# davelailai/DS-GCN

Hardware: AMD Instinct MI355X
Metric: clips/sec fwd+bwd, DS-STGCN NTU-60 3x64x25x2 (higher is better)
Workload: dtype f32

## Files before the change

ds-gcn_amd/csrc/tmsplit.hip:

```cpp
#include <algorithm>

#include "common.h"
#include "bn_jobs.h"

namespace {

constexpr int TS_NT = 256;
constexpr int TS_MAXBR = 8;
constexpr int TS_OOB = 0x7ffffff0;
constexpr int TS_R = 4, TS_H = 4;

typedef float f32x2s __attribute__((ext_vector_type(2)));
typedef unsigned u32x4s __attribute__((ext_vector_type(4)));

struct TSBranch {
  int type;
  int c0, bc, dil;
  const float* w;
  const float* b;
  float* dwp;
  float* dbp;
};

struct TSArgs {
  const float* z; const float* zaug; const float* scale; const float* shift;
  const float* coeff;
  float* f; float* oaug; float* stats;
  const float* ge; const float* doaug;
  float* dz; float* dzaug; float* part;
  int n_act, n, C, T, Tout, V, nbr, ngrp, ngrpa, nconv, eplanes, sboff, haw, splits, pstride;
  int cw[TS_MAXBR];
  int ngroups, gfirst[TS_MAXBR], gcount[TS_MAXBR];
  int exp;
  TSBranch br[TS_MAXBR];
};

__device__ __forceinline__ __amdgpu_buffer_rsrc_t ts_rsrc(const void* p, size_t bytes) {
  return __builtin_amdgcn_make_buffer_rsrc(const_cast<void*>(p), (short)0, (int)bytes, 0x00020000);
}
__device__ __forceinline__ f32x4 ts_load4(__amdgpu_buffer_rsrc_t r, int voff, int soff) {
  return __builtin_bit_cast(f32x4, __builtin_amdgcn_raw_buffer_load_b128(r, voff, soff, 0));
}
__device__ __forceinline__ f32x2s ts_load2(__amdgpu_buffer_rsrc_t r, int voff, int soff) {
  return __builtin_bit_cast(f32x2s, __builtin_amdgcn_raw_buffer_load_b64(r, voff, soff, 0));
}
__device__ __forceinline__ void ts_store4(f32x4 v, __amdgpu_buffer_rsrc_t r, int voff) {
  __builtin_amdgcn_raw_buffer_store_b128(__builtin_bit_cast(u32x4s, v), r, voff, 0, 0);
}
__device__ __forceinline__ int ts_row32(int r, int half) { return (r & 3) + 8 * (r >> 2) + 4 * half; }
__device__ __forceinline__ int ts_rowoff(bool ok, int base, int rowoff) {
  return (int)((unsigned)(ok ? base : TS_OOB) + (unsigned)rowoff);
}
__device__ __forceinline__ int ts_cp(int bc) { return (min(64, max(bc, 1)) + 7) & ~7; }

__device__ __forceinline__ const TSBranch& ts_conv_window(const TSArgs& a, int w) { return a.br[a.cw[w]]; }

template <typename ACC>
__device__ __forceinline__ ACC ts_rowread(const float* Tw, int half, int l31) {
  const f32x4* rowp = reinterpret_cast<const f32x4*>(Tw + l31 * 36 + half * 16);
  ACC s = 0;
#pragma unroll
  for (int q = 0; q < 4; ++q) {
    const f32x4 v = rowp[q];
    s += ((ACC)v.x + (ACC)v.y) + ((ACC)v.z + (ACC)v.w);
  }
  return s;
}


#ifdef DSGCN_LAB
__device__ long long g_tsc_stamp[16];
__device__ int g_tsc_block = 0;
#define TSC_STAMP() do { if (!AUG && (int)blockIdx.x == g_tsc_block && threadIdx.x == 0 && nst < 14) g_tsc_stamp[nst++] = wall_clock64(); } while (0)
#else
#define TSC_STAMP() do {} while (0)
#endif

template <bool FWD, int MT, bool ODD, bool AUG, bool S2 = false>
__device__ __forceinline__ void ts_conv(const TSArgs& a, const TSBranch& br, bool first, float* lds, int grp, int lane, int wave) {
  constexpr int KT = 3, PDK = 2, NS = KT * PDK;
  constexpr bool FOLD = FWD && !AUG;
  constexpr int FP = 32;
  static_assert(!(S2 && ODD), "stride 2 has its own load forms");
// ... 832 lines not shown
      if (a.br[i].type == 0)
        for (int k = lane; k < a.br[i].bc * 2; k += 64) tab[((size_t)(a.ngrp + n) * a.C + a.br[i].c0) * 2 + k] = 0.f;
  }
  const int per = S2 ? a.T * a.V + a.Tout * a.V + ((a.T + 3) & ~3) + ((a.Tout + 3) & ~3) + 32
                     : (FWD ? 1 : 2) * a.T * a.V + 2 * ((a.T + 3) & ~3) + 32;
  for (int i = 0; i < a.nbr; ++i) {
    if (a.br[i].type == 0) continue;
    if (c < a.br[i].bc) {
      if constexpr (S2) ts_elem2<FWD>(a, a.br[i], lds + (size_t)wave * per, n, c, lane);
      else ts_elem<FWD>(a, a.br[i], lds + (size_t)wave * per, n, c, lane);
      return;
    }
    c -= a.br[i].bc;
  }
}

__global__ __launch_bounds__(64) void k_tsp_prep(const float* __restrict__ gf, const float* __restrict__ f,
                                                 const float* __restrict__ oaug, const float* __restrict__ coeff,
                                                 const float* __restrict__ A0, const float* __restrict__ B0,
                                                 float* __restrict__ ge, float* __restrict__ doaug,
                                                 float* __restrict__ pcoef, int C, int T, int V) {
  extern __shared__ __attribute__((aligned(16))) float lds[];
  const int lane = threadIdx.x;
  const long plane = blockIdx.x;
  const int c = (int)(plane % C);
  const int L = T * V, L4n = L >> 2, Tp = (T + 3) & ~3;
  float* gl = lds;
  float* ol = lds + L;
  float* cf = ol + Tp;
  if (lane < V) cf[lane] = coeff[lane];
  for (int t = lane; t < T; t += 64) ol[t] = oaug[plane * T + t];
  const float a0 = A0 ? A0[c] : 0.f, b0 = B0 ? B0[c] : 0.f;
  const f32x4* g4 = gf ? reinterpret_cast<const f32x4*>(gf + plane * L) : nullptr;
  const f32x4* f4 = reinterpret_cast<const f32x4*>(f + plane * L);
  f32x4* o4 = reinterpret_cast<f32x4*>(ge + plane * L);
  f32x4* l4 = reinterpret_cast<f32x4*>(gl);
  const f32x4 zero4 = {0.f, 0.f, 0.f, 0.f};
  for (int base = 0; base < L4n; base += 256) {
    f32x4 gv[4], fv[4];
#pragma unroll
    for (int q = 0; q < 4; ++q) {
      const int i = base + q * 64 + lane;
      const bool ok = i < L4n;
      gv[q] = (ok && g4) ? g4[i] : zero4;
      fv[q] = (ok && A0) ? f4[i] : zero4;
    }
#pragma unroll
    for (int q = 0; q < 4; ++q) {
      const int i = base + q * 64 + lane;
      if (i < L4n) {
        f32x4 r;
#pragma unroll
        for (int k = 0; k < 4; ++k) r[k] = gv[q][k] + fmaf(b0, fv[q][k], a0);
        o4[i] = r;
        l4[i] = r;
      }
    }
  }
  wave_lds_sync();
  for (int t = lane; t < T; t += 64) {
    float acc = 0.f;
    for (int v = 0; v < V; ++v) acc = fmaf(gl[t * V + v], cf[v], acc);
    doaug[plane * T + t] = acc;
  }
  {
    const int v = lane & 31, hf = lane >> 5;
    float acc = 0.f;
    if (v < V)
      for (int t = hf; t < T; t += 2) acc = fmaf(gl[t * V + v], ol[t], acc);
    acc += __shfl_xor(acc, 32, 64);
    if (lane < V) pcoef[plane * V + lane] = acc;
  }
}

__host__ __device__ inline int tsw_ls(int w) { return ((w + 1) & ~3) + 2; }

#ifdef DSGCN_LAB
__device__ long long g_tsw_stamp[64];
#define TSW_STAMP() do { if (blockIdx.x == 0 && blockIdx.y == 0 && threadIdx.x == 0 && nst < 62) g_tsw_stamp[nst++] = wall_clock64(); } while (0)
#else
#define TSW_STAMP() do {} while (0)
#endif

template <int CH>
__global__ __launch_bounds__(TS_NT, CH == 32 ? 2 : 1) void k_tspw(TSArgs a, BnCoefTable jobs) {
  constexpr int KT = 3;
  constexpr int JD = CH == 32 ? 4 : 7, JX = CH == 32 ? 10 : 20;
  extern __shared__ __attribute__((aligned(16))) float lds[];
  if ((int)blockIdx.x >= a.splits) {
    if (blockIdx.y == 0)
      bnj_dispatch(jobs, (int)blockIdx.x - a.splits,
                   [&](const BnCoefJob& J, int b) { bn_coef_rows_block<TS_NT>(J, b, reinterpret_cast<double (*)[8][2]>(lds)); });
    return;
  }
#ifdef DSGCN_LAB
  int nst = 0;
#endif
  TSW_STAMP();
  const int tid = threadIdx.x, lane = tid & 63;
  const int wave = __builtin_amdgcn_readfirstlane(tid >> 6);
  const int half = lane >> 5, l31 = lane & 31;
  const int gw0 = a.gfirst[blockIdx.y], gcnt = a.gcount[blockIdx.y];
  const TSBranch& br = ts_conv_window(a, gw0);
  const int V = a.V, T = a.T, L = T * V, C = a.C;
  int bc = 0, ldil = br.dil;
  for (int w = 0; w < gcnt; ++w) {
    const TSBranch& bw = ts_conv_window(a, gw0 + w);
    if (l31 >= bc) ldil = bw.dil;
    bc += bw.bc;
  }
  const int GM = TS_R * V, XM = (TS_R + 2 * TS_H) * V;
  const int GS4 = GM >> 2, XS4 = XM >> 2, SEG4 = (TS_H * V) >> 2;
  const int LSd = tsw_ls(GM + TS_R), LSx = tsw_ls(XM + TS_R + 2 * TS_H);
  float* Ds = lds;
  float* Xs = lds + CH * LSd;
  f32x2s* SB = reinterpret_cast<f32x2s*>(Xs + CH * LSx);
  const f32x2s sb0 = (tid < CH && tid < bc) ? f32x2s{a.scale ? a.scale[br.c0 + tid] : 1.f, a.shift ? a.shift[br.c0 + tid] : 0.f}
                                            : f32x2s{0.f, 0.f};
  const int rel0 = br.c0;

  const int units = a.n * (T / TS_R);
  const int per = (units + a.splits - 1) / a.splits;
  const int u0 = blockIdx.x * per, u1 = min(units, u0 + per);

  const __amdgpu_buffer_rsrc_t rg = ts_rsrc(a.ge, (size_t)a.n * C * L * 4);
  const __amdgpu_buffer_rsrc_t rz = ts_rsrc(a.z, (size_t)a.n * C * L * 4);
  const __amdgpu_buffer_rsrc_t rga = ts_rsrc(a.doaug, (size_t)a.n * C * T * 4);
  const __amdgpu_buffer_rsrc_t rza = ts_rsrc(a.zaug, (size_t)a.n * C * T * 4);
  int vD[JD], lD[JD], vX[JX], lX[JX];
#pragma unroll
  for (int j = 0; j < JD; ++j) {
    const int f = tid + TS_NT * j, row = f / GS4, c4 = f - row * GS4;
    const bool ok = row < bc;
    vD[j] = ok ? (row * L + 4 * c4) * 4 : TS_OOB;
    lD[j] = ok ? row * LSd + 4 * c4 : -1;
  }
#pragma unroll
  for (int j = 0; j < JX; ++j) {
    const int f = tid + TS_NT * j, row = f / XS4, c4 = f - row * XS4;
    const bool ok = row < bc;
    vX[j] = ok ? (row * L + 4 * c4) * 4 : TS_OOB;
    const int seg = c4 / SEG4;
    lX[j] = (row * LSx + 4 * c4) | ((seg == 0 ? 1 : seg == 2 ? 2 : 0) << 20) | ((row & 63) << 22) | (ok ? 1 << 28 : 0);
  }
  const int arow = tid / 3, aseg = tid - arow * 3;
  const bool aokD = tid < CH && tid < bc && !(a.exp & 256), aokX = tid < 3 * CH && arow < bc && !(a.exp & 256);
  const int aneed = aseg == 0 ? 1 : aseg == 2 ? 2 : 0;
  f32x4 gr[JD], xr[JX], ga, xa;
  float dsum[JD], dsa = 0.f;
#pragma unroll
  for (int j = 0; j < JD; ++j) dsum[j] = 0.f;
  int inval = 0;
  auto issue = [&](int u) {
    const int n = u / (T / TS_R), t0 = (u - n * (T / TS_R)) * TS_R;
    const int sg = ((n * C + br.c0) * L + t0 * V) * 4;
    const int sx = ((n * C + br.c0) * L + (t0 - TS_H) * V) * 4;
    inval = (t0 >= TS_H ? 0 : 1) | (t0 + TS_R < T ? 0 : 2);
#pragma unroll
    for (int j = 0; j < JD; ++j) gr[j] = ts_load4(rg, vD[j], sg);
#pragma unroll
    for (int j = 0; j < JX; ++j) {
      const bool ok = (((lX[j] >> 20) & 3) & inval) == 0;
      xr[j] = ts_load4(rz, ok ? vX[j] + sx : TS_OOB, 0);
    }
    ga = ts_load4(rga, aokD ? ((n * C + br.c0 + tid) * T + t0) * 4 : TS_OOB, 0);
    const bool oka = aokX & ((aneed & inval) == 0);
    xa = ts_load4(rza, oka ? ((n * C + br.c0 + arow) * T + t0 + (aseg - 1) * TS_H) * 4 : TS_OOB, 0);
  };
  const bool noact = a.exp & 128;
  auto act = [&](float x, f32x2s sb, bool rl) -> float {
    if (noact) return x;
    const float y = fmaf(x, sb.x, sb.y);
    return rl ? fmaxf(y, 0.f) : y;
  };
  auto commit = [&]() {
#pragma unroll
    for (int j = 0; j < JD; ++j) {
      if (lD[j] >= 0) {
        f32x2s* d = reinterpret_cast<f32x2s*>(Ds + lD[j]);
        d[0] = f32x2s{gr[j].x, gr[j].y};
        d[1] = f32x2s{gr[j].z, gr[j].w};
        dsum[j] += (gr[j].x + gr[j].y) + (gr[j].z + gr[j].w);
      }
    }
#pragma unroll
    for (int j = 0; j < JX; ++j) {
      if (lX[j] & (1 << 28)) {
        const bool ok = (((lX[j] >> 20) & 3) & inval) == 0;
        const int row = (lX[j] >> 22) & 63;
        const f32x2s sb = SB[row];
        const bool rl = rel0 + row < a.n_act;
        f32x2s* d = reinterpret_cast<f32x2s*>(Xs + (lX[j] & 0xfffff));
        d[0] = ok ? f32x2s{act(xr[j].x, sb, rl), act(xr[j].y, sb, rl)} : f32x2s{0.f, 0.f};
        d[1] = ok ? f32x2s{act(xr[j].z, sb, rl), act(xr[j].w, sb, rl)} : f32x2s{0.f, 0.f};
      }
    }
    if (aokD) {
      f32x2s* d = reinterpret_cast<f32x2s*>(Ds + tid * LSd + GM);
      d[0] = f32x2s{ga.x, ga.y};
      d[1] = f32x2s{ga.z, ga.w};
      dsa += (ga.x + ga.y) + (ga.z + ga.w);
    }
    if (aokX) {
      const bool ok = (aneed & inval) == 0;
      const f32x2s sb = SB[arow];
      const bool rl = rel0 + arow < a.n_act;
      f32x2s* d = reinterpret_cast<f32x2s*>(Xs + arow * LSx + XM + aseg * TS_H);
      d[0] = ok ? f32x2s{act(xa.x, sb, rl), act(xa.y, sb, rl)} : f32x2s{0.f, 0.f};
      d[1] = ok ? f32x2s{act(xa.z, sb, rl), act(xa.w, sb, rl)} : f32x2s{0.f, 0.f};
    }
  };

  f32x16 acc[KT];
#pragma unroll
  for (int k = 0; k < KT; ++k)
#pragma unroll
    for (int i = 0; i < 16; ++i) acc[k][i] = 0.f;
  const int mt = CH == 64 ? (wave >> 1) : 0, nt = CH == 64 ? (wave & 1) : 0;
  const int g0 = CH == 32 ? (GS4 * wave) / 4 : 0, g1 = CH == 32 ? (GS4 * (wave + 1)) / 4 : GS4;
  const bool augw = CH == 64 || wave == 0;
  const int sh = ldil * V;
  const bool oddsh = gcnt > 1 || ((sh & 1) && !(a.exp & 512));
  const float* Ap = Ds + (32 * mt + l31) * LSd + 2 * half;
  const float* Bp = Xs + (32 * nt + l31) * LSx + TS_H * V + 2 * half;
  const float* Aq = Ds + (32 * mt + l31) * LSd + GM + 2 * half;
  const float* Bq = Xs + (32 * nt + l31) * LSx + XM + TS_H + 2 * half;
  auto mm = [&](f32x2s av, f32x2s b0, f32x2s b1, f32x2s b2) {
    acc[0] = __builtin_amdgcn_mfma_f32_32x32x2f32(av.x, b0.x, acc[0], 0, 0, 0);
    acc[1] = __builtin_amdgcn_mfma_f32_32x32x2f32(av.x, b1.x, acc[1], 0, 0, 0);
    acc[2] = __builtin_amdgcn_mfma_f32_32x32x2f32(av.x, b2.x, acc[2], 0, 0, 0);
    acc[0] = __builtin_amdgcn_mfma_f32_32x32x2f32(av.y, b0.y, acc[0], 0, 0, 0);
    acc[1] = __builtin_amdgcn_mfma_f32_32x32x2f32(av.y, b1.y, acc[1], 0, 0, 0);
    acc[2] = __builtin_amdgcn_mfma_f32_32x32x2f32(av.y, b2.y, acc[2], 0, 0, 0);
  };

  if (u0 < u1) issue(u0);
  {
    f32x4* l4 = reinterpret_cast<f32x4*>(lds);
    for (int i = tid; i < (CH * (LSd + LSx)) >> 2; i += TS_NT) l4[i] = f32x4{0.f, 0.f, 0.f, 0.f};
    if (tid < CH) SB[tid] = sb0;
  }
  __syncthreads();
  TSW_STAMP();
  for (int u = u0; u < u1; ++u) {
    commit();
    asm volatile("s_waitcnt lgkmcnt(0)" ::: "memory");
    __builtin_amdgcn_s_barrier();
    TSW_STAMP();
    if (u + 1 < u1) issue(u + 1);
    TSW_STAMP();
    if (oddsh) {
#pragma unroll 2
      for (int g = g0; g < g1; ++g) {
        const f32x2s av = *reinterpret_cast<const f32x2s*>(Ap + 4 * g);
        const f32x2s b1 = *reinterpret_cast<const f32x2s*>(Bp + 4 * g);
        const f32x2s b0 = {Bp[4 * g - sh], Bp[4 * g - sh + 1]};
        const f32x2s b2 = {Bp[4 * g + sh], Bp[4 * g + sh + 1]};
        mm(av, b0, b1, b2);
      }
    } else {
#pragma unroll 2
      for (int g = g0; g < g1; ++g) {
        const f32x2s av = *reinterpret_cast<const f32x2s*>(Ap + 4 * g);
        const f32x2s b0 = *reinterpret_cast<const f32x2s*>(Bp + 4 * g - sh);
        const f32x2s b1 = *reinterpret_cast<const f32x2s*>(Bp + 4 * g);
        const f32x2s b2 = *reinterpret_cast<const f32x2s*>(Bp + 4 * g + sh);
        mm(av, b0, b1, b2);
      }
    }
    if (augw) {
      const f32x2s av = *reinterpret_cast<const f32x2s*>(Aq);
      const f32x2s b1 = *reinterpret_cast<const f32x2s*>(Bq);
      const f32x2s b0 = {Bq[-ldil], Bq[1 - ldil]};
      const f32x2s b2 = {Bq[ldil], Bq[1 + ldil]};
      mm(av, b0, b1, b2);
    }
    asm volatile("s_waitcnt lgkmcnt(0)" ::: "memory");
    __builtin_amdgcn_s_barrier();
    TSW_STAMP();
  }

  if (CH == 32) {
    float* Rs = lds;
#pragma unroll
    for (int k = 0; k < KT; ++k)
#pragma unroll
      for (int r = 0; r < 16; ++r) Rs[((wave * KT + k) * 32 + ts_row32(r, half)) * 33 + l31] = acc[k][r];
    __syncthreads();
    for (int w = 0, r0 = 0; w < gcnt; ++w) {
      const TSBranch& bw = ts_conv_window(a, gw0 + w);
      const int wb = bw.bc;
      float* dw = bw.dwp + (size_t)blockIdx.x * a.pstride;
      for (int o = tid; o < KT * wb * wb; o += TS_NT) {
        const int co = o / (wb * KT), r2 = o - co * wb * KT, ci = r2 / KT, k = r2 - ci * KT;
        float v = 0.f;
#pragma unroll
        for (int wv = 0; wv < 4; ++wv) v += Rs[((wv * KT + k) * 32 + r0 + co) * 33 + r0 + ci];
        dw[o] = v;
      }
      r0 += wb;
    }
    __syncthreads();
  } else {
    float* dw = br.dwp + (size_t)blockIdx.x * a.pstride;
    const int ci = 32 * nt + l31;
    if (ci < bc) {
#pragma unroll
      for (int r = 0; r < 16; ++r) {
        const int co = 32 * mt + ts_row32(r, half);
        if (co < bc) {
#pragma unroll
          for (int k = 0; k < KT; ++k) dw[((size_t)co * bc + ci) * KT + k] = acc[k][r];
        }
      }
    }
    __syncthreads();
  }
  float* Bs = lds;
#pragma unroll
  for (int j = 0; j < JD; ++j) {
    const int f = tid + TS_NT * j, row = f / GS4, c4 = f - row * GS4;
    if (row < bc) Bs[row * (GS4 + 2) + c4] = dsum[j];
  }
  if (aokD) Bs[tid * (GS4 + 2) + GS4] = dsa;
  __syncthreads();
  if (tid < bc) {
    float v = 0.f;
    for (int c = 0; c <= GS4; ++c) v += Bs[tid * (GS4 + 2) + c];
    int r0 = 0;
    for (int w = 0; w < gcnt; ++w) {
      const TSBranch& bw = ts_conv_window(a, gw0 + w);
      if (tid >= r0 && tid < r0 + bw.bc) bw.dbp[(size_t)blockIdx.x * a.pstride + tid - r0] = v;
      r0 += bw.bc;
    }
  }
#ifdef DSGCN_LAB
  TSW_STAMP();
  if (blockIdx.x == 0 && blockIdx.y == 0 && threadIdx.x == 0) g_tsw_stamp[63] = nst;
#endif
}

template <int CH>
__global__ __launch_bounds__(TS_NT, CH == 32 ? 2 : 1) void k_tspw2(TSArgs a, BnCoefTable jobs) {
  constexpr int KT = 3;
  constexpr int JD = CH == 32 ? 4 : 7, JX = CH == 32 ? 11 : 21, JA = CH == 32 ? 2 : 3;
  extern __shared__ __attribute__((aligned(16))) float lds[];
  if ((int)blockIdx.x >= a.splits) {
    if (blockIdx.y == 0)
      bnj_dispatch(jobs, (int)blockIdx.x - a.splits,
                   [&](const BnCoefJob& J, int b) { bn_coef_rows_block<TS_NT>(J, b, reinterpret_cast<double (*)[8][2]>(lds)); });
    return;
  }
  const int tid = threadIdx.x, lane = tid & 63;
  const int wave = __builtin_amdgcn_readfirstlane(tid >> 6);
  const int half = lane >> 5, l31 = lane & 31;
  const int gw0 = a.gfirst[blockIdx.y], gcnt = a.gcount[blockIdx.y];
  const TSBranch& br = ts_conv_window(a, gw0);
  const int V = a.V, Ti = a.T, To = a.Tout, Li = Ti * V, Lo = To * V, C = a.C;
  int bc = 0;
  for (int w = 0; w < gcnt; ++w) bc += ts_conv_window(a, gw0 + w).bc;
  auto row_dil = [&](int row) -> int {
    int d = br.dil, r0 = 0;
    for (int w = 0; w < gcnt; ++w) {
      const TSBranch& bw = ts_conv_window(a, gw0 + w);
      if (row >= r0) d = bw.dil;
      r0 += bw.bc;
    }
    return d;
  };
  const int GM = TS_R * V;
  const int GS4 = GM >> 2, Q = (V + 3) >> 2;
  const int LSd = tsw_ls(GM + TS_R);
  float* Ds = lds;
  float* Xs = lds + CH * LSd;
  f32x2s* SB = reinterpret_cast<f32x2s*>(Xs + 3 * CH * LSd);
  const f32x2s sb0 = (tid < CH && tid < bc) ? f32x2s{a.scale ? a.scale[br.c0 + tid] : 1.f, a.shift ? a.shift[br.c0 + tid] : 0.f}
                                            : f32x2s{0.f, 0.f};
  const int rel0 = br.c0;
  const int units = a.n * (To / TS_R);
  const int per = (units + a.splits - 1) / a.splits;
  const int u0 = blockIdx.x * per, u1 = min(units, u0 + per);
  const __amdgpu_buffer_rsrc_t rg = ts_rsrc(a.ge, (size_t)a.n * C * Lo * 4);
  const __amdgpu_buffer_rsrc_t rz = ts_rsrc(a.z, (size_t)a.n * C * Li * 4);
  const __amdgpu_buffer_rsrc_t rga = ts_rsrc(a.doaug, (size_t)a.n * C * To * 4);
  const __amdgpu_buffer_rsrc_t rza = ts_rsrc(a.zaug, (size_t)a.n * C * Ti * 4);
  int vD[JD], lD[JD];
#pragma unroll
  for (int j = 0; j < JD; ++j) {
    const int f = tid + TS_NT * j, row = f / GS4, c4 = f - row * GS4;
    const bool ok = row < bc;
    vD[j] = ok ? (row * Lo + 4 * c4) * 4 : TS_OOB;
    lD[j] = ok ? row * LSd + 4 * c4 : -1;
  }
  int vX[JX], lX[JX], fX[JX];
#pragma unroll
  for (int j = 0; j < JX; ++j) {
    const int f = tid + TS_NT * j, row = f / (12 * Q), r1 = f - row * 12 * Q, tap = r1 / (4 * Q), r2 = r1 - tap * 4 * Q,
              fr = r2 / Q, q = r2 - fr * Q;
    const bool ok = row < bc;
    const int fo = 2 * fr + (tap - 1) * row_dil(row);
    fX[j] = fo;
    vX[j] = ok ? (row * Li + fo * V + 4 * q) * 4 : TS_OOB;
    lX[j] = ((tap * CH + row) * LSd + fr * V + 4 * q) | (min(4, V - 4 * q) << 20) | ((row & 63) << 23) | (ok ? 1 << 29 : 0);
  }
  const bool aokD = tid < CH && tid < bc;
  int vA[JA], lA[JA], fA[JA];
#pragma unroll
// ... 93 lines not shown
    for (int i = tid; i < (4 * CH * LSd) >> 2; i += TS_NT) l4[i] = f32x4{0.f, 0.f, 0.f, 0.f};
    if (tid < CH) SB[tid] = sb0;
  }
  __syncthreads();
  for (int u = u0; u < u1; ++u) {
    commit();
    asm volatile("s_waitcnt lgkmcnt(0)" ::: "memory");
    __builtin_amdgcn_s_barrier();
    if (u + 1 < u1) issue(u + 1);
#pragma unroll 2
    for (int g = g0; g < g1; ++g) {
      const f32x2s av = *reinterpret_cast<const f32x2s*>(Ap + 4 * g);
      const f32x2s b0 = *reinterpret_cast<const f32x2s*>(Bp + 4 * g);
      const f32x2s b1 = *reinterpret_cast<const f32x2s*>(Bp + CH * LSd + 4 * g);
      const f32x2s b2 = *reinterpret_cast<const f32x2s*>(Bp + 2 * CH * LSd + 4 * g);
      acc[0] = __builtin_amdgcn_mfma_f32_32x32x2f32(av.x, b0.x, acc[0], 0, 0, 0);
      acc[1] = __builtin_amdgcn_mfma_f32_32x32x2f32(av.x, b1.x, acc[1], 0, 0, 0);
      acc[2] = __builtin_amdgcn_mfma_f32_32x32x2f32(av.x, b2.x, acc[2], 0, 0, 0);
      acc[0] = __builtin_amdgcn_mfma_f32_32x32x2f32(av.y, b0.y, acc[0], 0, 0, 0);
      acc[1] = __builtin_amdgcn_mfma_f32_32x32x2f32(av.y, b1.y, acc[1], 0, 0, 0);
      acc[2] = __builtin_amdgcn_mfma_f32_32x32x2f32(av.y, b2.y, acc[2], 0, 0, 0);
    }
    asm volatile("s_waitcnt lgkmcnt(0)" ::: "memory");
    __builtin_amdgcn_s_barrier();
  }
  if (CH == 32) {
    float* Rs = lds;
#pragma unroll
    for (int k = 0; k < KT; ++k)
#pragma unroll
      for (int r = 0; r < 16; ++r) Rs[((wave * KT + k) * 32 + ts_row32(r, half)) * 33 + l31] = acc[k][r];
    __syncthreads();
    for (int w = 0, r0 = 0; w < gcnt; ++w) {
      const TSBranch& bw = ts_conv_window(a, gw0 + w);
      const int wb = bw.bc;
      float* dw = bw.dwp + (size_t)blockIdx.x * a.pstride;
      for (int o = tid; o < KT * wb * wb; o += TS_NT) {
        const int co = o / (wb * KT), r2 = o - co * wb * KT, ci = r2 / KT, k = r2 - ci * KT;
        float v = 0.f;
#pragma unroll
        for (int wv = 0; wv < 4; ++wv) v += Rs[((wv * KT + k) * 32 + r0 + co) * 33 + r0 + ci];
        dw[o] = v;
      }
      r0 += wb;
    }
    __syncthreads();
  } else {
    float* dw = br.dwp + (size_t)blockIdx.x * a.pstride;
    const int ci = 32 * nt + l31;
    if (ci < bc) {
#pragma unroll
      for (int r = 0; r < 16; ++r) {
        const int co = 32 * mt + ts_row32(r, half);
        if (co < bc) {
#pragma unroll
          for (int k = 0; k < KT; ++k) dw[((size_t)co * bc + ci) * KT + k] = acc[k][r];
        }
      }
    }
    __syncthreads();
  }
  float* Bs = lds;
#pragma unroll
  for (int j = 0; j < JD; ++j) {
    const int f = tid + TS_NT * j, row = f / GS4, c4 = f - row * GS4;
    if (row < bc) Bs[row * (GS4 + 2) + c4] = dsum[j];
  }
  if (aokD) Bs[tid * (GS4 + 2) + GS4] = dsa;
  __syncthreads();
  if (tid < bc) {
    float v = 0.f;
    for (int c = 0; c <= GS4; ++c) v += Bs[tid * (GS4 + 2) + c];
    int r0 = 0;
    for (int w = 0; w < gcnt; ++w) {
      const TSBranch& bw = ts_conv_window(a, gw0 + w);
      if (tid >= r0 && tid < r0 + bw.bc) bw.dbp[(size_t)blockIdx.x * a.pstride + tid - r0] = v;
      r0 += bw.bc;
    }
  }
}

int g_ts_exp = 0;
constexpr size_t TS_LDS_MAX = 156 * 1024;

template <typename F>
int ts_raise_lds(F* kernel, size_t lds, size_t* have) {
  if (lds > TS_LDS_MAX) return DSGCN_EUNSUPPORTED;
  if (lds > *have) {
    hipError_t e = hipFuncSetAttribute((const void*)kernel, hipFuncAttributeMaxDynamicSharedMemorySize, (int)TS_LDS_MAX);
    if (e != hipSuccess) return (int)e;
    *have = TS_LDS_MAX;
  }
  return 0;
}

int ts_fill(TSArgs& a, int n, int C, int T, int V, int stride, int KT, int nbr, const int* type, const int* c0,
            const int* bc, const int* dil) {
  if (n <= 0 || C <= 0 || T <= 0 || V <= 0 || nbr <= 0 || nbr > TS_MAXBR || !type || !c0 || !bc || !dil) return DSGCN_EINVAL;
  a.n = n; a.C = C; a.T = T; a.V = V; a.nbr = nbr; a.exp = g_ts_exp;
  a.Tout = stride == 2 ? T / 2 : T;
  int nconv = 0, eplanes = 0, wmax = 0, next = 0;
  for (int i = 0; i < nbr; ++i) {
    TSBranch& b = a.br[i];
    b.type = type[i]; b.c0 = c0[i]; b.bc = bc[i]; b.dil = dil[i];
    if (b.bc <= 0 || b.c0 != next) return b.bc <= 0 ? DSGCN_EINVAL : 0;
    next += b.bc;
    if (b.type == 0) {
      a.cw[nconv] = i;
      ++nconv;
      wmax = std::max(wmax, b.bc);
      if (b.dil < 1 || b.dil > TS_H) return 0;
    } else if (b.type == 1 || b.type == 2) {
      eplanes += b.bc;
    } else {
      return DSGCN_EINVAL;
    }
  }
  if (next != C) return 0;
  if (KT != 3 || (stride != 1 && stride != 2) || nconv == 0 || wmax > 64 || (V & 1) == 0 || V < 5 || V > 25 || T % 4 ||
      (long)T * V > 2048)
    return 0;
  if (stride == 2 && (T % 8 || T > 128)) return 0;
  const long L = (long)T * V;
  if ((long)n * C * L * 4 >= (1L << 31) - 4096 || (long)n * L >= (1L << 31) - 256) return 0;
  if (n > 32768) return 0;
  a.nconv = nconv;
  a.eplanes = eplanes;
  a.ngroups = 0;
  for (int i = 0, k = 0, prev = -2, gsum = 0; i < nbr; ++i) {
    if (a.br[i].type != 0) continue;
    if (a.ngroups > 0 && prev == i - 1 && wmax <= 32 && gsum + a.br[i].bc <= 32) {
      ++a.gcount[a.ngroups - 1];
      gsum += a.br[i].bc;
    } else {
      a.gfirst[a.ngroups] = k;
      a.gcount[a.ngroups] = 1;
      ++a.ngroups;
      gsum = a.br[i].bc;
    }
    prev = i;
    ++k;
  }
  a.haw = 32;
  while (a.haw < (511 / V + 2) * stride + 2 * TS_H + 3) a.haw *= 2;
  return wmax <= 32 ? 1 : 2;
}

void ts_groups(TSArgs& a, bool fwd) {
  const int Tt = fwd ? a.Tout : a.T;
  a.ngrp = (int)(((long)a.n * Tt * a.V + 511) / 512);
  a.ngrpa = (int)(((long)a.n * Tt + 511) / 512);
}

size_t ts_lds_main(TSArgs& a, int MT, bool fwd) {
  int cpmax = 8;
  for (int i = 0; i < a.nbr; ++i)
    if (a.br[i].type == 0) cpmax = std::max(cpmax, (std::min(64, a.br[i].bc) + 7) & ~7);
  const size_t wsf = (size_t)64 * (3 * cpmax + 1) + 64;
  const size_t epf = (size_t)4 * 32 * 36 + (size_t)4 * MT * 32 * 2 * 2;
  const size_t convf = (std::max(wsf, epf) + 3) & ~(size_t)3;
  a.sboff = (int)convf;
  const size_t planef = a.Tout != a.T ? (size_t)4 * (a.T * a.V + a.Tout * a.V + ((a.T + 3) & ~3) + ((a.Tout + 3) & ~3) + 32)
                                      : (size_t)4 * ((fwd ? 1 : 2) * a.T * a.V + 2 * ((a.T + 3) & ~3) + 32);
  return std::max(convf + 192 + (fwd ? (size_t)64 * a.haw : 0), planef) * sizeof(float);
}

template <bool FWD>
int ts_launch_main(TSArgs& a, int MT, hipStream_t st) {
  const size_t lds = ts_lds_main(a, MT, FWD);
  ts_groups(a, FWD);
  const long blocks = (long)a.nconv * (a.ngrp + a.ngrpa) + ((long)a.n * a.eplanes + 3) / 4;
  if (blocks <= 0 || blocks >= (1L << 31)) return DSGCN_EUNSUPPORTED;
  const dim3 grid((unsigned)blocks), blk(TS_NT);
  if (a.Tout != a.T) {
// ... 56 lines not shown
    return std::min(splits, units);
  }
  return 0;
}

int dsgcn_tms_split_fwd(const float* z, const float* zaug, const float* scale, const float* shift, int n_act,
                        const float* coeff, float* f, float* oaug, float* stats, int n, int C, int T, int V, int stride,
                        int nbr, const int* type, const int* c0, const int* bc, const int* dil, const float* const* w,
                        const float* const* b, void* stream) {
  if (!z || !zaug || !coeff || !f || !oaug || !w) return DSGCN_EINVAL;
  TSArgs a = {};
  const int mt = ts_fill(a, n, C, T, V, stride, 3, nbr, type, c0, bc, dil);
  if (mt < 0) return mt;
  if (mt == 0) return DSGCN_EUNSUPPORTED;
  a.z = z; a.zaug = zaug; a.scale = scale; a.shift = shift; a.n_act = n_act; a.coeff = coeff;
  a.f = f; a.oaug = oaug; a.stats = stats;
  for (int i = 0; i < nbr; ++i) {
    a.br[i].w = w[i]; a.br[i].b = b ? b[i] : nullptr;
    if (type[i] == 0 && !a.br[i].w) return DSGCN_EINVAL;
  }
  hipStream_t st = (hipStream_t)stream;
  return ts_launch_main<true>(a, mt, st);
}

int dsgcn_tms_split_prep(const float* gf, const float* f, const float* oaug, const float* coeff, const float* A0,
                         const float* B0, float* ge, float* doaug, float* pcoef, int n, int C, int T, int V,
                         void* stream) {
  if (!f || !oaug || !coeff || !ge || !doaug || !pcoef || n <= 0 || C <= 0 || T <= 0 || V <= 0) return DSGCN_EINVAL;
  if ((T * V) % 4 || V > 32 || (A0 && !B0)) return DSGCN_EUNSUPPORTED;
  const size_t lds = ((size_t)T * V + ((T + 3) & ~3) + 32) * sizeof(float);
  if (lds > 64 * 1024) return DSGCN_EUNSUPPORTED;
  hipLaunchKernelGGL(k_tsp_prep, dim3((unsigned)((long)n * C)), dim3(64), lds, (hipStream_t)stream, gf, f, oaug, coeff,
                     A0, B0, ge, doaug, pcoef, C, T, V);
  DSGCN_LAUNCH_CHECK();
  return 0;
}

int dsgcn_tms_split_dgrad(const float* z, const float* zaug, const float* scale, const float* shift, int n_act,
                          const float* ge, const float* doaug, float* dz, float* dzaug, float* part, int n, int C, int T,
                          int V, int stride, int nbr, const int* type, const int* c0, const int* bc, const int* dil,
                          const float* const* w, void* stream) {
  if (!z || !zaug || !ge || !doaug || !dz || !dzaug || !part || !w) return DSGCN_EINVAL;
  TSArgs a = {};
  const int mt = ts_fill(a, n, C, T, V, stride, 3, nbr, type, c0, bc, dil);
  if (mt < 0) return mt;
  if (mt == 0) return DSGCN_EUNSUPPORTED;
  a.z = z; a.zaug = zaug; a.scale = scale; a.shift = shift; a.n_act = n_act;
  a.ge = ge; a.doaug = doaug; a.dz = dz; a.dzaug = dzaug; a.part = part;
  for (int i = 0; i < nbr; ++i) {
    a.br[i].w = w[i];
    if (type[i] == 0 && !a.br[i].w) return DSGCN_EINVAL;
  }
  hipStream_t st = (hipStream_t)stream;
  return ts_launch_main<false>(a, mt, st);
}

int dsgcn_tms_split_wgrad_jobs(const float* z, const float* zaug, const float* scale, const float* shift, int n_act,
                               const float* ge, const float* doaug, int n, int C, int T, int V, int stride, int nbr,
                               const int* type, const int* c0, const int* bc, const int* dil, float* const* dwp,
                               float* const* dbp, int splits, int pstride, const dsgcn_bn_coef_job* jobs, int njobs,
                               void* stream) {
  if (!z || !zaug || !ge || !doaug || !dwp || !dbp || splits <= 0) return DSGCN_EINVAL;
  if (njobs < 0 || njobs > BNJ_MAX || (njobs > 0 && !jobs)) return DSGCN_EINVAL;
  BnCoefTable jt = {};
  jt.n = njobs;
  for (int i = 0; i < njobs; ++i) {
    const dsgcn_bn_coef_job& q = jobs[i];
    jt.j[i] = BnCoefJob{q.part, q.mean, q.var, q.gamma, q.coef, q.count, q.eps, q.R, q.C, q.k, q.i_ds, q.i_dh, q.c_affine,
                        q.accumulate};
  }
  if (!bnj_coef_ok(jt)) return DSGCN_EINVAL;
  TSArgs a = {};
  const int mt = ts_fill(a, n, C, T, V, stride, 3, nbr, type, c0, bc, dil);
  if (mt < 0) return mt;
  if (mt == 0) return DSGCN_EUNSUPPORTED;
  a.z = z; a.zaug = zaug; a.scale = scale; a.shift = shift; a.n_act = n_act;
  a.ge = ge; a.doaug = doaug; a.splits = splits; a.pstride = pstride;
  for (int i = 0; i < nbr; ++i) {
    a.br[i].dwp = dwp[i]; a.br[i].dbp = dbp[i];
    if (type[i] == 0 && (!a.br[i].dwp || !a.br[i].dbp)) return DSGCN_EINVAL;
  }
  const int ch = mt == 1 ? 32 : 64;
  const size_t tile = stride == 2 ? (size_t)4 * ch * tsw_ls(TS_R * (V + 1)) + 2 * ch
                                  : (size_t)ch * (tsw_ls(TS_R * (V + 1)) + tsw_ls((TS_R + 2 * TS_H) * (V + 1))) + 2 * ch;
  const size_t red = (size_t)4 * 3 * 32 * 33;
  const size_t lds = std::max(tile, ch == 32 ? red : (size_t)0) * sizeof(float);
  const dim3 grid((unsigned)(splits + bnj_total_blocks(jt)), (unsigned)a.ngroups);
  if (stride == 2) {
    if (ch == 32) {
      static size_t have = 64 * 1024;
      const int rc = ts_raise_lds(k_tspw2<32>, lds, &have);
      if (rc) return rc;
      hipLaunchKernelGGL(k_tspw2<32>, grid, dim3(TS_NT), lds, (hipStream_t)stream, a, jt);
    } else {
      static size_t have = 64 * 1024;
      const int rc = ts_raise_lds(k_tspw2<64>, lds, &have);
      if (rc) return rc;
      hipLaunchKernelGGL(k_tspw2<64>, grid, dim3(TS_NT), lds, (hipStream_t)stream, a, jt);
    }
  } else if (ch == 32) {
    static size_t have = 64 * 1024;
    const int rc = ts_raise_lds(k_tspw<32>, lds, &have);
    if (rc) return rc;
    hipLaunchKernelGGL(k_tspw<32>, grid, dim3(TS_NT), lds, (hipStream_t)stream, a, jt);
  } else {
    static size_t have = 64 * 1024;
    const int rc = ts_raise_lds(k_tspw<64>, lds, &have);
    if (rc) return rc;
    hipLaunchKernelGGL(k_tspw<64>, grid, dim3(TS_NT), lds, (hipStream_t)stream, a, jt);
  }
  DSGCN_LAUNCH_CHECK();
  return 0;
}

int dsgcn_tms_split_wgrad(const float* z, const float* zaug, const float* scale, const float* shift, int n_act,
                          const float* ge, const float* doaug, int n, int C, int T, int V, int stride, int nbr,
                          const int* type, const int* c0, const int* bc, const int* dil, float* const* dwp, float* const* dbp,
                          int splits, int pstride, void* stream) {
  return dsgcn_tms_split_wgrad_jobs(z, zaug, scale, shift, n_act, ge, doaug, n, C, T, V, stride, nbr, type, c0, bc, dil, dwp,
                                    dbp, splits, pstride, nullptr, 0, stream);
}

}
```

Before: 5910.

## Reuse input halo via ring buffer and double-buffer gradient tiles in temporal wgrad

Reworks the stride-1 temporal-conv weight-gradient kernel so the activated input window lives in a 16-row circular buffer in LDS. Each step loads only the next 4-row segment instead of re-fetching the full 12-row halo window, and the full window is reloaded only when a new sample starts. Gradient tiles are double-buffered so the next unit's loads and commit overlap the MFMA work on the current one. The cost is more LDS, wrap-around index arithmetic in the inner loop, and extra barriers at sample boundaries.

Measured after the change: 5912, median of 6. About the same (+0.0%).

```diff
diff --git a/ds-gcn_amd/csrc/tmsplit.hip b/ds-gcn_amd/csrc/tmsplit.hip
--- a/ds-gcn_amd/csrc/tmsplit.hip
+++ b/ds-gcn_amd/csrc/tmsplit.hip
@@ -1,4 +1,5 @@
 #include <algorithm>
+#include <type_traits>
 
 #include "common.h"
 #include "bn_jobs.h"
@@ -997,10 +998,12 @@
 #define TSW_STAMP() do {} while (0)
 #endif
 
+constexpr int TSW_RF = 16;
+
 template <int CH>
-__global__ __launch_bounds__(TS_NT, CH == 32 ? 2 : 1) void k_tspw(TSArgs a, BnCoefTable jobs) {
+__global__ __launch_bounds__(TS_NT, CH == 32 ? 2 : 1) void k_tsw1(TSArgs a, BnCoefTable jobs) {
   constexpr int KT = 3;
-  constexpr int JD = CH == 32 ? 4 : 7, JX = CH == 32 ? 10 : 20;
+  constexpr int JD = CH == 32 ? 4 : 7;
   extern __shared__ __attribute__((aligned(16))) float lds[];
   if ((int)blockIdx.x >= a.splits) {
     if (blockIdx.y == 0)
@@ -1024,17 +1027,17 @@
     if (l31 >= bc) ldil = bw.dil;
     bc += bw.bc;
   }
-  const int GM = TS_R * V, XM = (TS_R + 2 * TS_H) * V;
-  const int GS4 = GM >> 2, XS4 = XM >> 2, SEG4 = (TS_H * V) >> 2;
-  const int LSd = tsw_ls(GM + TS_R), LSx = tsw_ls(XM + TS_R + 2 * TS_H);
+  const int GM = TS_R * V, GS4 = GM >> 2, RM = TSW_RF * V;
+  const int LSd = tsw_ls(GM + TS_R), LSr = tsw_ls(RM + TSW_RF);
   float* Ds = lds;
-  float* Xs = lds + CH * LSd;
-  f32x2s* SB = reinterpret_cast<f32x2s*>(Xs + CH * LSx);
+  float* Xs = lds + 2 * CH * LSd;
+  f32x2s* SB = reinterpret_cast<f32x2s*>(Xs + CH * LSr);
   const f32x2s sb0 = (tid < CH && tid < bc) ? f32x2s{a.scale ? a.scale[br.c0 + tid] : 1.f, a.shift ? a.shift[br.c0 + tid] : 0.f}
                                             : f32x2s{0.f, 0.f};
   const int rel0 = br.c0;
 
-  const int units = a.n * (T / TS_R);
+  const int upn = T / TS_R;
+  const int units = a.n * upn;
   const int per = (units + a.splits - 1) / a.splits;
   const int u0 = blockIdx.x * per, u1 = min(units, u0 + per);
 
@@ -1042,45 +1045,42 @@
   const __amdgpu_buffer_rsrc_t rz = ts_rsrc(a.z, (size_t)a.n * C * L * 4);
   const __amdgpu_buffer_rsrc_t rga = ts_rsrc(a.doaug, (size_t)a.n * C * T * 4);
   const __amdgpu_buffer_rsrc_t rza = ts_rsrc(a.zaug, (size_t)a.n * C * T * 4);
-  int vD[JD], lD[JD], vX[JX], lX[JX];
+  int vS[JD], lD[JD], lX[JD];
 #pragma unroll
   for (int j = 0; j < JD; ++j) {
     const int f = tid + TS_NT * j, row = f / GS4, c4 = f - row * GS4;
     const bool ok = row < bc;
-    vD[j] = ok ? (row * L + 4 * c4) * 4 : TS_OOB;
+    vS[j] = ok ? (row * L + 4 * c4) * 4 : TS_OOB;
     lD[j] = ok ? row * LSd + 4 * c4 : -1;
-  }
-#pragma unroll
-  for (int j = 0; j < JX; ++j) {
-    const int f = tid + TS_NT * j, row = f / XS4, c4 = f - row * XS4;
-    const bool ok = row < bc;
-    vX[j] = ok ? (row * L + 4 * c4) * 4 : TS_OOB;
-    const int seg = c4 / SEG4;
-    lX[j] = (row * LSx + 4 * c4) | ((seg == 0 ? 1 : seg == 2 ? 2 : 0) << 20) | ((row & 63) << 22) | (ok ? 1 << 28 : 0);
-  }
-  const int arow = tid / 3, aseg = tid - arow * 3;
-  const bool aokD = tid < CH && tid < bc && !(a.exp & 256), aokX = tid < 3 * CH && arow < bc && !(a.exp & 256);
-  const int aneed = aseg == 0 ? 1 : aseg == 2 ? 2 : 0;
-  f32x4 gr[JD], xr[JX], ga, xa;
+    lX[j] = (row & 63) * LSr + 4 * c4;
+  }
+  const bool aok = tid < CH && tid < bc && !(a.exp & 256);
+  const bool rla = rel0 + tid < a.n_act;
+  f32x4 gr[JD], xr[3][JD], ga, xa[3];
   float dsum[JD], dsa = 0.f;
 #pragma unroll
   for (int j = 0; j < JD; ++j) dsum[j] = 0.f;
-  int inval = 0;
-  auto issue = [&](int u) {
-    const int n = u / (T / TS_R), t0 = (u - n * (T / TS_R)) * TS_R;
-    const int sg = ((n * C + br.c0) * L + t0 * V) * 4;
-    const int sx = ((n * C + br.c0) * L + (t0 - TS_H) * V) * 4;
-    inval = (t0 >= TS_H ? 0 : 1) | (t0 + TS_R < T ? 0 : 2);
-#pragma unroll
-    for (int j = 0; j < JD; ++j) gr[j] = ts_load4(rg, vD[j], sg);
-#pragma unroll
-    for (int j = 0; j < JX; ++j) {
-      const bool ok = (((lX[j] >> 20) & 3) & inval) == 0;
-      xr[j] = ts_load4(rz, ok ? vX[j] + sx : TS_OOB, 0);
-    }
-    ga = ts_load4(rga, aokD ? ((n * C + br.c0 + tid) * T + t0) * 4 : TS_OOB, 0);
-    const bool oka = aokX & ((aneed & inval) == 0);
-    xa = ts_load4(rza, oka ? ((n * C + br.c0 + arow) * T + t0 + (aseg - 1) * TS_H) * 4 : TS_OOB, 0);
+  int sn = 0, sk = 0;
+  bool sfresh = true;
+  auto seg_ok = [&](int i) { const int s = sk - 1 + i; return s >= 0 && s < upn; };
+  auto issue = [&](int u, bool fresh) {
+    sn = u / upn;
+    sk = u - sn * upn;
+    sfresh = fresh;
+    const int t0 = sk * TS_R;
+    const int sg = ((sn * C + br.c0) * L + t0 * V) * 4;
+#pragma unroll
+    for (int j = 0; j < JD; ++j) gr[j] = ts_load4(rg, vS[j], sg);
+    ga = ts_load4(rga, aok ? ((sn * C + br.c0 + tid) * T + t0) * 4 : TS_OOB, 0);
+#pragma unroll
+    for (int i = 0; i < 3; ++i) {
+      if (i < 2 && !fresh) continue;
+      const bool ok = seg_ok(i);
+      const int sx = ((sn * C + br.c0) * L + (t0 + (i - 1) * TS_R) * V) * 4;
+#pragma unroll
+      for (int j = 0; j < JD; ++j) xr[i][j] = ts_load4(rz, (ok && lD[j] >= 0) ? vS[j] + sx : TS_OOB, 0);
+      xa[i] = ts_load4(rza, (ok && aok) ? ((sn * C + br.c0 + tid) * T + t0 + (i - 1) * TS_R) * 4 : TS_OOB, 0);
+    }
   };
   const bool noact = a.exp & 128;
   auto act = [&](float x, f32x2s sb, bool rl) -> float {
@@ -1088,41 +1088,45 @@
     const float y = fmaf(x, sb.x, sb.y);
     return rl ? fmaxf(y, 0.f) : y;
   };
-  auto commit = [&]() {
+  auto commit = [&](int buf) {
+    float* D = Ds + buf * CH * LSd;
 #pragma unroll
     for (int j = 0; j < JD; ++j) {
       if (lD[j] >= 0) {
-        f32x2s* d = reinterpret_cast<f32x2s*>(Ds + lD[j]);
+        f32x2s* d = reinterpret_cast<f32x2s*>(D + lD[j]);
         d[0] = f32x2s{gr[j].x, gr[j].y};
         d[1] = f32x2s{gr[j].z, gr[j].w};
         dsum[j] += (gr[j].x + gr[j].y) + (gr[j].z + gr[j].w);
       }
     }
-#pragma unroll
-    for (int j = 0; j < JX; ++j) {
-      if (lX[j] & (1 << 28)) {
-        const bool ok = (((lX[j] >> 20) & 3) & inval) == 0;
-        const int row = (lX[j] >> 22) & 63;
-        const f32x2s sb = SB[row];
-        const bool rl = rel0 + row < a.n_act;
-        f32x2s* d = reinterpret_cast<f32x2s*>(Xs + (lX[j] & 0xfffff));
-        d[0] = ok ? f32x2s{act(xr[j].x, sb, rl), act(xr[j].y, sb, rl)} : f32x2s{0.f, 0.f};
-        d[1] = ok ? f32x2s{act(xr[j].z, sb, rl), act(xr[j].w, sb, rl)} : f32x2s{0.f, 0.f};
-      }
-    }
-    if (aokD) {
-      f32x2s* d = reinterpret_cast<f32x2s*>(Ds + tid * LSd + GM);
+    if (aok) {
+      f32x2s* d = reinterpret_cast<f32x2s*>(D + tid * LSd + GM);
       d[0] = f32x2s{ga.x, ga.y};
       d[1] = f32x2s{ga.z, ga.w};
       dsa += (ga.x + ga.y) + (ga.z + ga.w);
     }
-    if (aokX) {
-      const bool ok = (aneed & inval) == 0;
-      const f32x2s sb = SB[arow];
-      const bool rl = rel0 + arow < a.n_act;
-      f32x2s* d = reinterpret_cast<f32x2s*>(Xs + arow * LSx + XM + aseg * TS_H);
-      d[0] = ok ? f32x2s{act(xa.x, sb, rl), act(xa.y, sb, rl)} : f32x2s{0.f, 0.f};
-      d[1] = ok ? f32x2s{act(xa.z, sb, rl), act(xa.w, sb, rl)} : f32x2s{0.f, 0.f};
+#pragma unroll
+    for (int i = 0; i < 3; ++i) {
+      if (i < 2 && !sfresh) continue;
+      const bool ok = seg_ok(i);
+      const int pos = (sk - 1 + i) & 3;
+#pragma unroll
+      for (int j = 0; j < JD; ++j) {
+        if (lD[j] >= 0) {
+          const int row = (tid + TS_NT * j) / GS4;
+          const f32x2s sb = SB[row];
+          const bool rl = rel0 + row < a.n_act;
+          f32x2s* d = reinterpret_cast<f32x2s*>(Xs + lX[j] + pos * GM);
+          d[0] = ok ? f32x2s{act(xr[i][j].x, sb, rl), act(xr[i][j].y, sb, rl)} : f32x2s{0.f, 0.f};
+          d[1] = ok ? f32x2s{act(xr[i][j].z, sb, rl), act(xr[i][j].w, sb, rl)} : f32x2s{0.f, 0.f};
+        }
+      }
+      if (aok) {
+        const f32x2s sb = SB[tid];
+        f32x2s* d = reinterpret_cast<f32x2s*>(Xs + tid * LSr + RM + 4 * pos);
+        d[0] = ok ? f32x2s{act(xa[i].x, sb, rla), act(xa[i].y, sb, rla)} : f32x2s{0.f, 0.f};
+        d[1] = ok ? f32x2s{act(xa[i].z, sb, rla), act(xa[i].w, sb, rla)} : f32x2s{0.f, 0.f};
+      }
     }
   };
 
@@ -1135,11 +1139,10 @@
   const int g0 = CH == 32 ? (GS4 * wave) / 4 : 0, g1 = CH == 32 ? (GS4 * (wave + 1)) / 4 : GS4;
   const bool augw = CH == 64 || wave == 0;
   const int sh = ldil * V;
-  const bool oddsh = gcnt > 1 || ((sh & 1) && !(a.exp & 512));
+  const bool oddsh = __builtin_amdgcn_readfirstlane(gcnt > 1 || ((sh & 1) && !(a.exp & 512)));
   const float* Ap = Ds + (32 * mt + l31) * LSd + 2 * half;
-  const float* Bp = Xs + (32 * nt + l31) * LSx + TS_H * V + 2 * half;
-  const float* Aq = Ds + (32 * mt + l31) * LSd + GM + 2 * half;
-  const float* Bq = Xs + (32 * nt + l31) * LSx + XM + TS_H + 2 * half;
+  const float* Br = Xs + (32 * nt + l31) * LSr;
+  const float* Bq = Br + RM;
   auto mm = [&](f32x2s av, f32x2s b0, f32x2s b1, f32x2s b2) {
     acc[0] = __builtin_amdgcn_mfma_f32_32x32x2f32(av.x, b0.x, acc[0], 0, 0, 0);
     acc[1] = __builtin_amdgcn_mfma_f32_32x32x2f32(av.x, b1.x, acc[1], 0, 0, 0);
@@ -1149,47 +1152,71 @@
     acc[2] = __builtin_amdgcn_mfma_f32_32x32x2f32(av.y, b2.y, acc[2], 0, 0, 0);
   };
 
-  if (u0 < u1) issue(u0);
+  if (u0 < u1) issue(u0, true);
   {
     f32x4* l4 = reinterpret_cast<f32x4*>(lds);
-    for (int i = tid; i < (CH * (LSd + LSx)) >> 2; i += TS_NT) l4[i] = f32x4{0.f, 0.f, 0.f, 0.f};
+    for (int i = tid; i < (CH * (2 * LSd + LSr)) >> 2; i += TS_NT) l4[i] = f32x4{0.f, 0.f, 0.f, 0.f};
     if (tid < CH) SB[tid] = sb0;
   }
   __syncthreads();
+  if (u0 < u1) commit(u0 & 1);
+  asm volatile("s_waitcnt lgkmcnt(0)" ::: "memory");
+  __builtin_amdgcn_s_barrier();
   TSW_STAMP();
   for (int u = u0; u < u1; ++u) {
-    commit();
-    asm volatile("s_waitcnt lgkmcnt(0)" ::: "memory");
-    __builtin_amdgcn_s_barrier();
+    const bool nxt = u + 1 < u1;
+    const bool fresh = nxt && (u + 1) % upn == 0;
+    const int k = u % upn;
+    if (nxt) issue(u + 1, fresh);
     TSW_STAMP();
-    if (u + 1 < u1) issue(u + 1);
+    const float* A = Ap + (u & 1) * CH * LSd;
+    const int x0 = (k & 3) * GM + 2 * half;
+    auto products = [&](auto odd) {
+      auto opnd = [&](int g, f32x2s& av, f32x2s& b0, f32x2s& b1, f32x2s& b2) {
+        const int xc = x0 + 4 * g;
+        int xm = xc - sh, xp = xc + sh;
+        xm += xm < 0 ? RM : 0;
+        xp -= xp >= RM ? RM : 0;
+        av = *reinterpret_cast<const f32x2s*>(A + 4 * g);
+        b1 = *reinterpret_cast<const f32x2s*>(Br + xc);
+        if constexpr (decltype(odd)::value) {
+          const int xm1 = xm + 1 == RM ? 0 : xm + 1, xp1 = xp + 1 == RM ? 0 : xp + 1;
+          b0 = f32x2s{Br[xm], Br[xm1]};
+          b2 = f32x2s{Br[xp], Br[xp1]};
+        } else {
+          b0 = *reinterpret_cast<const f32x2s*>(Br + xm);
+          b2 = *reinterpret_cast<const f32x2s*>(Br + xp);
+        }
+      };
+      if (g0 < g1) {
+        f32x2s av, b0, b1, b2;
+        opnd(g0, av, b0, b1, b2);
+        for (int g = g0; g < g1; ++g) {
+          f32x2s nav, nb0, nb1, nb2;
+          opnd(g + 1 < g1 ? g + 1 : g, nav, nb0, nb1, nb2);
+          mm(av, b0, b1, b2);
+          av = nav; b0 = nb0; b1 = nb1; b2 = nb2;
+        }
+      }
+    };
+    if (oddsh)
+      products(std::true_type{});
+    else
+      products(std::false_type{});
+    if (augw) {
+      const int y = (k & 3) * TS_R + 2 * half;
+      const f32x2s av = *reinterpret_cast<const f32x2s*>(A + GM);
+      const f32x2s b1 = *reinterpret_cast<const f32x2s*>(Bq + y);
+      const f32x2s b0 = {Bq[(y - ldil) & (TSW_RF - 1)], Bq[(y + 1 - ldil) & (TSW_RF - 1)]};
+      const f32x2s b2 = {Bq[(y + ldil) & (TSW_RF - 1)], Bq[(y + 1 + ldil) & (TSW_RF - 1)]};
+      mm(av, b0, b1, b2);
+    }
     TSW_STAMP();
-    if (oddsh) {
-#pragma unroll 2
-      for (int g = g0; g < g1; ++g) {
-        const f32x2s av = *reinterpret_cast<const f32x2s*>(Ap + 4 * g);
-        const f32x2s b1 = *reinterpret_cast<const f32x2s*>(Bp + 4 * g);
-        const f32x2s b0 = {Bp[4 * g - sh], Bp[4 * g - sh + 1]};
-        const f32x2s b2 = {Bp[4 * g + sh], Bp[4 * g + sh + 1]};
-        mm(av, b0, b1, b2);
-      }
-    } else {
-#pragma unroll 2
-      for (int g = g0; g < g1; ++g) {
-        const f32x2s av = *reinterpret_cast<const f32x2s*>(Ap + 4 * g);
-        const f32x2s b0 = *reinterpret_cast<const f32x2s*>(Bp + 4 * g - sh);
-        const f32x2s b1 = *reinterpret_cast<const f32x2s*>(Bp + 4 * g);
-        const f32x2s b2 = *reinterpret_cast<const f32x2s*>(Bp + 4 * g + sh);
-        mm(av, b0, b1, b2);
-      }
-    }
-    if (augw) {
-      const f32x2s av = *reinterpret_cast<const f32x2s*>(Aq);
-      const f32x2s b1 = *reinterpret_cast<const f32x2s*>(Bq);
-      const f32x2s b0 = {Bq[-ldil], Bq[1 - ldil]};
-      const f32x2s b2 = {Bq[ldil], Bq[1 + ldil]};
-      mm(av, b0, b1, b2);
-    }
+    if (fresh) {
+      asm volatile("s_waitcnt lgkmcnt(0)" ::: "memory");
+      __builtin_amdgcn_s_barrier();
+    }
+    if (nxt) commit((u + 1) & 1);
     asm volatile("s_waitcnt lgkmcnt(0)" ::: "memory");
     __builtin_amdgcn_s_barrier();
     TSW_STAMP();
@@ -1237,7 +1264,7 @@
     const int f = tid + TS_NT * j, row = f / GS4, c4 = f - row * GS4;
     if (row < bc) Bs[row * (GS4 + 2) + c4] = dsum[j];
   }
-  if (aokD) Bs[tid * (GS4 + 2) + GS4] = dsa;
+  if (aok) Bs[tid * (GS4 + 2) + GS4] = dsa;
   __syncthreads();
   if (tid < bc) {
     float v = 0.f;
@@ -1497,14 +1524,15 @@
 
 int g_ts_exp = 0;
 constexpr size_t TS_LDS_MAX = 156 * 1024;
+constexpr size_t TSW_LDS_MAX = 160 * 1024;
 
 template <typename F>
-int ts_raise_lds(F* kernel, size_t lds, size_t* have) {
-  if (lds > TS_LDS_MAX) return DSGCN_EUNSUPPORTED;
+int ts_raise_lds(F* kernel, size_t lds, size_t* have, size_t cap = TS_LDS_MAX) {
+  if (lds > cap) return DSGCN_EUNSUPPORTED;
   if (lds > *have) {
-    hipError_t e = hipFuncSetAttribute((const void*)kernel, hipFuncAttributeMaxDynamicSharedMemorySize, (int)TS_LDS_MAX);
+    hipError_t e = hipFuncSetAttribute((const void*)kernel, hipFuncAttributeMaxDynamicSharedMemorySize, (int)cap);
     if (e != hipSuccess) return (int)e;
-    *have = TS_LDS_MAX;
+    *have = cap;
   }
   return 0;
 }
@@ -1727,7 +1755,7 @@
   }
   const int ch = mt == 1 ? 32 : 64;
   const size_t tile = stride == 2 ? (size_t)4 * ch * tsw_ls(TS_R * (V + 1)) + 2 * ch
-                                  : (size_t)ch * (tsw_ls(TS_R * (V + 1)) + tsw_ls((TS_R + 2 * TS_H) * (V + 1))) + 2 * ch;
+                                  : (size_t)ch * (2 * tsw_ls(TS_R * (V + 1)) + tsw_ls(TSW_RF * (V + 1))) + 2 * ch;
   const size_t red = (size_t)4 * 3 * 32 * 33;
   const size_t lds = std::max(tile, ch == 32 ? red : (size_t)0) * sizeof(float);
   const dim3 grid((unsigned)(splits + bnj_total_blocks(jt)), (unsigned)a.ngroups);
@@ -1745,14 +1773,14 @@
     }
   } else if (ch == 32) {
     static size_t have = 64 * 1024;
-    const int rc = ts_raise_lds(k_tspw<32>, lds, &have);
+    const int rc = ts_raise_lds(k_tsw1<32>, lds, &have, TSW_LDS_MAX);
     if (rc) return rc;
-    hipLaunchKernelGGL(k_tspw<32>, grid, dim3(TS_NT), lds, (hipStream_t)stream, a, jt);
+    hipLaunchKernelGGL(k_tsw1<32>, grid, dim3(TS_NT), lds, (hipStream_t)stream, a, jt);
   } else {
     static size_t have = 64 * 1024;
-    const int rc = ts_raise_lds(k_tspw<64>, lds, &have);
+    const int rc = ts_raise_lds(k_tsw1<64>, lds, &have, TSW_LDS_MAX);
     if (rc) return rc;
-    hipLaunchKernelGGL(k_tspw<64>, grid, dim3(TS_NT), lds, (hipStream_t)stream, a, jt);
+    hipLaunchKernelGGL(k_tsw1<64>, grid, dim3(TS_NT), lds, (hipStream_t)stream, a, jt);
   }
   DSGCN_LAUNCH_CHECK();
   return 0;
```
